# yflyl613/Tiny-NewsRec

Hardware: AMD Instinct MI355X
Metric: training impressions/sec (higher is better)
Workload: dtype fp16; 1 GPU; Tiny-NewsRec 4-layer student (train [2, 3]) + 4-teacher KD (title-emb MSE + soft-CE), fwd+bwd+AMSGrad; batch_per_gpu=32, global_batch=32, user_log_length=50, candidates=5, num_words_title=30, news_dim=256, n_news=51282, parallelism=dp1

## Files before the change

### tiny-newsrec_amd/csrc/attn.hip

```cpp
#include "common.h"

namespace {

constexpr float NEG_BIG = -3.0e38f;
#ifndef TNR_ATTN_TS
#define TNR_ATTN_TS 144
#endif
constexpr int TS = TNR_ATTN_TS;
constexpr int TB = 32 * TS;

__device__ __forceinline__ f32x16 zero16() {
    f32x16 z;
#pragma unroll
    for (int r = 0; r < 16; ++r) z[r] = 0.f;
    return z;
}

__device__ __forceinline__ bf16x8 cat4(bf16x4 a, bf16x4 b) { return __builtin_shufflevector(a, b, 0, 1, 2, 3, 4, 5, 6, 7); }

__device__ __forceinline__ bf16x8 tr_frag(const char* tile, int s, int ct, int lane) {
    const int g16 = lane >> 4, hh = g16 >> 1, i16 = lane & 15, q = i16 >> 2, p = i16 & 3;
    const int row = 16 * s + 4 * hh + q;
    const int col = ct * 32 + 16 * (g16 & 1) + 4 * p;
    bf16x4 v0 = ds_read_tr16(tile + row * TS + col * 2);
    bf16x4 v1 = ds_read_tr16(tile + (row + 8) * TS + col * 2);
    return cat4(v0, v1);
}

__device__ __forceinline__ void acc_to_frags(const f32x16& x, bf16x8 (&f)[2]) {
#pragma unroll
    for (int s = 0; s < 2; ++s)
#pragma unroll
        for (int jj = 0; jj < 8; ++jj) f[s][jj] = (bf16)x[8 * s + jj];
}

__device__ __forceinline__ void acc_to_lds(char* tile, const f32x16& x, int ct, int lane, float scale) {
    const int h = lane >> 5, c = ct * 32 + (lane & 31);
#pragma unroll
    for (int r = 0; r < 16; ++r) {
        int row = (r & 3) + 8 * (r >> 2) + 4 * h;
        *(bf16*)(tile + row * TS + c * 2) = (bf16)(x[r] * scale);
    }
}

__global__ __launch_bounds__(256) void attn_fwd_kernel(const bf16* __restrict__ qkv, const float* __restrict__ mask_add,
                                                       const float* __restrict__ rel, bf16* __restrict__ ctx,
                                                       int64_t n_pairs, int L, int A, TnrDrop drop) {
    __shared__ __attribute__((aligned(16))) char lds[4][TB];
    const int lane = threadIdx.x & 63, w = threadIdx.x >> 6;
    int64_t pair = (int64_t)blockIdx.x * 4 + w;
    const bool valid = pair < n_pairs;
    if (!valid) pair = n_pairs - 1;
    const int64_t n = pair / A;
    const int a = (int)(pair - n * A);
    const int HD = A * 64;
    const int64_t ldq = 3 * HD;
    const int row = lane & 31, h = lane >> 5;
    const int rowc = row < L ? row : L - 1;
    char* my = lds[w];

    f32x4 mkv[4], rlv[4];
    {
        const float* relp0 = rel + a * 1024 + row * 32;
        const float* mp0 = mask_add + n * 32;
#pragma unroll
        for (int g = 0; g < 4; ++g) {
            mkv[g] = *(const f32x4*)(mp0 + 8 * g + 4 * h);
            rlv[g] = *(const f32x4*)(relp0 + 8 * g + 4 * h);
        }
    }
    const bf16* qp = qkv + (n * L + rowc) * ldq + a * 64 + 8 * h;
    bf16x8 qf[4], kf[4];
#pragma unroll
    for (int s = 0; s < 4; ++s) {
        qf[s] = *(const bf16x8*)(qp + 16 * s);
        kf[s] = *(const bf16x8*)(qp + HD + 16 * s);
    }
#pragma unroll
    for (int p = 0; p < 4; ++p) {
        int idx = p * 64 + lane, r = idx >> 3, c = idx & 7;
        int rc = r < L ? r : L - 1;
        *(bf16x8*)(my + r * TS + c * 16) = *(const bf16x8*)(qkv + (n * L + rc) * ldq + 2 * HD + a * 64 + c * 8);
    }
    f32x16 st = zero16();
#pragma unroll
    for (int s = 0; s < 4; ++s) st = TNR_MFMA_32x32x16(kf[s], qf[s], st, 0, 0, 0);

    float mx = NEG_BIG;
#pragma unroll
    for (int g = 0; g < 4; ++g) {
        const f32x4 mk = mkv[g], rl = rlv[g];
#pragma unroll
        for (int e = 0; e < 4; ++e) {
            float v = st[4 * g + e] * 0.125f + mk[e] + rl[e];
            st[4 * g + e] = v;
            mx = fmaxf(mx, v);
        }
    }
    mx = fmaxf(mx, __shfl_xor(mx, 32, 64));
    float sum = 0.f;
#pragma unroll
    for (int r = 0; r < 16; ++r) {
        st[r] = __expf(st[r] - mx);
        sum += st[r];
    }
    sum += __shfl_xor(sum, 32, 64);
    const float inv = 1.0f / sum;
#pragma unroll
    for (int r = 0; r < 16; ++r) st[r] *= inv;
    if (drop.thresh) {
#pragma unroll
        for (int g = 0; g < 4; ++g) {
            float dm[4];
            tnr_drop_prob_row(drop, (uint64_t)pair, 8, row, 8 * g + 4 * h, dm);
#pragma unroll
            for (int e = 0; e < 4; ++e) st[4 * g + e] *= dm[e];
        }
    }
    bf16x8 pf[2];
    acc_to_frags(st, pf);

    f32x16 o[2];
#pragma unroll
    for (int ct = 0; ct < 2; ++ct) {
        o[ct] = zero16();
#pragma unroll
        for (int s = 0; s < 2; ++s)
            o[ct] = TNR_MFMA_32x32x16(pf[s], tr_frag(my, s, ct, lane), o[ct], 0, 0, 0);
    }
    acc_to_lds(my, o[0], 0, lane, 1.0f);
    acc_to_lds(my, o[1], 1, lane, 1.0f);
#pragma unroll
    for (int p = 0; p < 4; ++p) {
        int idx = p * 64 + lane, r = idx >> 3, c = idx & 7;
        if (valid && r < L) *(bf16x8*)(ctx + (n * L + r) * HD + a * 64 + c * 8) = *(const bf16x8*)(my + r * TS + c * 16);
    }
}

__global__ __launch_bounds__(256, 2) void attn_bwd_kernel(const bf16* __restrict__ qkv, const float* __restrict__ mask_add,
                                                       const float* __restrict__ rel, const bf16* __restrict__ dctx,
                                                       bf16* __restrict__ dqkv, float* __restrict__ bias_part,
                                                       int64_t n_pairs, int L, int A, TnrDrop drop) {
    __shared__ __attribute__((aligned(16))) char lds[4][3 * TB + 256];
    const int lane = threadIdx.x & 63, w = threadIdx.x >> 6;
    int64_t pair = (int64_t)blockIdx.x * 4 + w;
    const bool valid = pair < n_pairs;
    if (!valid) pair = n_pairs - 1;
    const int64_t n = pair / A;
    const int a = (int)(pair - n * A);
    const int HD = A * 64;
    const int64_t ldq = 3 * HD;
    const int row = lane & 31, h = lane >> 5;
    const int rowc = row < L ? row : L - 1;
    char* tK = lds[w];
    char* tO = tK + TB;
    char* tQ = tK + 2 * TB;
    float* stat = (float*)(tK + 3 * TB);

    f32x4 mkv[4], rlv[4];
    float relcol[16];
    const float* mp = mask_add + n * 32;
    const float mkcol = mp[row];
    {
        const float* relp0 = rel + a * 1024 + row * 32;
        const float* relc0 = rel + a * 1024 + row;
#pragma unroll
        for (int g = 0; g < 4; ++g) {
            mkv[g] = *(const f32x4*)(mp + 8 * g + 4 * h);
            rlv[g] = *(const f32x4*)(relp0 + 8 * g + 4 * h);
#pragma unroll
            for (int e = 0; e < 4; ++e) relcol[4 * g + e] = relc0[(8 * g + 4 * h + e) * 32];
        }
    }
    const bf16* qp = qkv + (n * L + rowc) * ldq + a * 64 + 8 * h;
    const bf16* dop = dctx + (n * L + rowc) * HD + a * 64 + 8 * h;
    bf16x8 qf[4], kf[4], vf[4], df[4];
#pragma unroll
    for (int s = 0; s < 4; ++s) {
        qf[s] = *(const bf16x8*)(qp + 16 * s);
        kf[s] = *(const bf16x8*)(qp + HD + 16 * s);
        vf[s] = *(const bf16x8*)(qp + 2 * HD + 16 * s);
        df[s] = *(const bf16x8*)(dop + 16 * s);
        if (row >= L) {
#pragma unroll
            for (int e = 0; e < 8; ++e) df[s][e] = (bf16)0.f;
        }
        int off = row * TS + (16 * s + 8 * h) * 2;
        *(bf16x8*)(tK + off) = kf[s];
        *(bf16x8*)(tO + off) = df[s];
        *(bf16x8*)(tQ + off) = qf[s];
    }

    f32x16 st = zero16(), dpt = zero16();
#pragma unroll
    for (int s = 0; s < 4; ++s) {
        st = TNR_MFMA_32x32x16(kf[s], qf[s], st, 0, 0, 0);
        dpt = TNR_MFMA_32x32x16(vf[s], df[s], dpt, 0, 0, 0);
    }
    {
        float mx = NEG_BIG;
#pragma unroll
        for (int g = 0; g < 4; ++g) {
            const f32x4 mk = mkv[g], rl = rlv[g];
#pragma unroll
            for (int e = 0; e < 4; ++e) {
                float v = st[4 * g + e] * 0.125f + mk[e] + rl[e];
                st[4 * g + e] = v;
                mx = fmaxf(mx, v);
            }
        }
        mx = fmaxf(mx, __shfl_xor(mx, 32, 64));
        float sum = 0.f;
#pragma unroll
        for (int r = 0; r < 16; ++r) {
            st[r] = __expf(st[r] - mx);
            sum += st[r];
        }
        sum += __shfl_xor(sum, 32, 64);
        const float inv = 1.0f / sum;
        float dsum = 0.f;
        if (drop.thresh) {
#pragma unroll
            for (int g = 0; g < 4; ++g) {
                float dm[4];
                tnr_drop_prob_row(drop, (uint64_t)pair, 8, row, 8 * g + 4 * h, dm);
#pragma unroll
                for (int e = 0; e < 4; ++e) dpt[4 * g + e] *= dm[e];
            }
        }
#pragma unroll
        for (int r = 0; r < 16; ++r) {
            st[r] *= inv;
            dsum += st[r] * dpt[r];
        }
        dsum += __shfl_xor(dsum, 32, 64);
        if (h == 0) {
            stat[row] = mx + __logf(sum);
            stat[32 + row] = dsum;
        }
#pragma unroll
        for (int r = 0; r < 16; ++r) st[r] = st[r] * (dpt[r] - dsum);
    }
    bf16x8 dstf[2];
    acc_to_frags(st, dstf);
    f32x16 dq[2];
#pragma unroll
    for (int ct = 0; ct < 2; ++ct) {
        dq[ct] = zero16();
#pragma unroll
        for (int s = 0; s < 2; ++s)
            dq[ct] = TNR_MFMA_32x32x16(dstf[s], tr_frag(tK, s, ct, lane), dq[ct], 0, 0, 0);
    }

    f32x16 sn = zero16(), dpn = zero16();
#pragma unroll
    for (int s = 0; s < 4; ++s) {
        sn = TNR_MFMA_32x32x16(qf[s], kf[s], sn, 0, 0, 0);
        dpn = TNR_MFMA_32x32x16(df[s], vf[s], dpn, 0, 0, 0);
    }
    {
        const float mk = mkcol;
#pragma unroll
        for (int g = 0; g < 4; ++g) {
            f32x4 lse = *(const f32x4*)(stat + 8 * g + 4 * h);
            f32x4 dd = *(const f32x4*)(stat + 32 + 8 * g + 4 * h);
            float dm[4] = {1.f, 1.f, 1.f, 1.f};
            if (drop.thresh) tnr_drop_prob_col(drop, (uint64_t)pair, 8, 8 * g + 4 * h, row, dm);
#pragma unroll
            for (int e = 0; e < 4; ++e) {
                float p = __expf(sn[4 * g + e] * 0.125f + mk + relcol[4 * g + e] - lse[e]);
                sn[4 * g + e] = p * dm[e];
                float dpm;
                {
#pragma clang fp contract(off)
                    dpm = dpn[4 * g + e] * dm[e];
                }
                dpn[4 * g + e] = p * (dpm - dd[e]);
            }
        }
    }
    bf16x8 pnf[2], dsf[2];
    acc_to_frags(sn, pnf);
    acc_to_frags(dpn, dsf);
    f32x16 dv[2], dk[2];
#pragma unroll
    for (int ct = 0; ct < 2; ++ct) {
        dv[ct] = zero16();
        dk[ct] = zero16();
#pragma unroll
        for (int s = 0; s < 2; ++s) {
            dv[ct] = TNR_MFMA_32x32x16(pnf[s], tr_frag(tO, s, ct, lane), dv[ct], 0, 0, 0);
            dk[ct] = TNR_MFMA_32x32x16(dsf[s], tr_frag(tQ, s, ct, lane), dk[ct], 0, 0, 0);
        }
    }
    if (bias_part != nullptr && valid) {
        float* bp = bias_part + n * ldq + a * 64 + (lane & 31);
#pragma unroll
        for (int ct = 0; ct < 2; ++ct) {
            float sq = 0.f, sk = 0.f, sv = 0.f;
#pragma unroll
            for (int r = 0; r < 16; ++r) {
                sq += (float)(bf16)(dq[ct][r] * 0.125f);
                sk += (float)(bf16)(dk[ct][r] * 0.125f);
                sv += (float)(bf16)dv[ct][r];
            }
            sq += __shfl_xor(sq, 32, 64);
            sk += __shfl_xor(sk, 32, 64);
            sv += __shfl_xor(sv, 32, 64);
            if (h == 0) {
                bp[ct * 32] = sq;
                bp[HD + ct * 32] = sk;
                bp[2 * HD + ct * 32] = sv;
            }
        }
    }
    acc_to_lds(tK, dq[0], 0, lane, 0.125f);
    acc_to_lds(tK, dq[1], 1, lane, 0.125f);
    acc_to_lds(tO, dk[0], 0, lane, 0.125f);
    acc_to_lds(tO, dk[1], 1, lane, 0.125f);
    acc_to_lds(tQ, dv[0], 0, lane, 1.0f);
    acc_to_lds(tQ, dv[1], 1, lane, 1.0f);
#pragma unroll
    for (int p = 0; p < 4; ++p) {
        int idx = p * 64 + lane, r = idx >> 3, c = idx & 7;
        if (valid && r < L) {
            bf16* dst = dqkv + (n * L + r) * ldq + a * 64 + c * 8;
            *(bf16x8*)(dst) = *(const bf16x8*)(tK + r * TS + c * 16);
            *(bf16x8*)(dst + HD) = *(const bf16x8*)(tO + r * TS + c * 16);
            *(bf16x8*)(dst + 2 * HD) = *(const bf16x8*)(tQ + r * TS + c * 16);
        }
    }
}

__device__ __forceinline__ bf16x8 ld_frag(const bf16* base, int64_t ld, int row, int h, int s) {
    return *(const bf16x8*)(base + (int64_t)row * ld + 16 * s + 8 * h);
}

__global__ __launch_bounds__(256, 3) void attn_long_fwd_kernel(const bf16* __restrict__ qkv, const float* __restrict__ mask_add,
                                                            const float* __restrict__ rel, bf16* __restrict__ ctx,
                                                            float* __restrict__ lse, int64_t n_items, int L, int Lr, int A,
                                                            TnrDrop drop) {
    __shared__ __attribute__((aligned(16))) char sk[2][TB], sv[2][TB], so[4][TB];
    const int tid = threadIdx.x, lane = tid & 63, w = tid >> 6;
    const int nqt = Lr >> 5, nqg = (nqt + 3) >> 2;
    const int qg = (int)(blockIdx.x % nqg);
    const int64_t na = blockIdx.x / nqg;
    (void)n_items;
    const int64_t n = na / A;
    const int a = (int)(na - n * A);
    const int qt_raw = qg * 4 + w;
    const bool valid = qt_raw < nqt;
    const int qt = valid ? qt_raw : nqt - 1;
    const int HD = A * 64;
    const int64_t ldq = 3 * HD;
    const int row = lane & 31, h = lane >> 5;
    char* my = so[w];
    const int qi = qt * 32 + row;
    const int qic = qi < L ? qi : L - 1;
    const bf16* qbase = qkv + (n * L) * ldq + a * 64;
    bf16x8 qf[4];
#pragma unroll
    for (int s = 0; s < 4; ++s) qf[s] = ld_frag(qbase, ldq, qic, h, s);
    f32x16 o[2] = {zero16(), zero16()};
    float m_run = NEG_BIG, l_run = 0.f;
    const float* relq = rel + ((int64_t)a * Lr + (qi < Lr ? qi : Lr - 1)) * Lr;
    const float* mp = mask_add + n * Lr;
    const int lr = tid >> 3, lc = tid & 7;
    bf16x8 kreg, vreg;
    auto gload = [&](int kt) {
        int rc = kt * 32 + lr;
        rc = rc < L ? rc : L - 1;
        kreg = *(const bf16x8*)(qbase + HD + (int64_t)rc * ldq + lc * 8);
        vreg = *(const bf16x8*)(qbase + 2 * HD + (int64_t)rc * ldq + lc * 8);
    };
    f32x4 mkn[4], rln[4];
    auto aload = [&](int kt) {
#pragma unroll
        for (int g = 0; g < 4; ++g) {
            mkn[g] = *(const f32x4*)(mp + kt * 32 + 8 * g + 4 * h);
            rln[g] = *(const f32x4*)(relq + kt * 32 + 8 * g + 4 * h);
        }
    };
    gload(0);
    aload(0);
    for (int kt = 0; kt < nqt; ++kt) {
        const int cur = kt & 1;
        *(bf16x8*)(sk[cur] + lr * TS + lc * 16) = kreg;
        *(bf16x8*)(sv[cur] + lr * TS + lc * 16) = vreg;
        f32x4 mkc[4], rlc[4];
#pragma unroll
        for (int g = 0; g < 4; ++g) { mkc[g] = mkn[g]; rlc[g] = rln[g]; }
        __syncthreads();
        if (kt + 1 < nqt) { gload(kt + 1); aload(kt + 1); }
        bf16x8 kf[4];
#pragma unroll
        for (int s = 0; s < 4; ++s) kf[s] = *(const bf16x8*)(sk[cur] + row * TS + (16 * s + 8 * h) * 2);
        f32x16 st = zero16();
#pragma unroll
        for (int s = 0; s < 4; ++s) st = TNR_MFMA_32x32x16(kf[s], qf[s], st, 0, 0, 0);
        float mx = NEG_BIG;
#pragma unroll
        for (int g = 0; g < 4; ++g) {
            const f32x4 mk = mkc[g], rl = rlc[g];
#pragma unroll
            for (int e = 0; e < 4; ++e) {
                float v = st[4 * g + e] * 0.125f + mk[e] + rl[e];
                st[4 * g + e] = v;
                mx = fmaxf(mx, v);
            }
        }
        mx = fmaxf(mx, __shfl_xor(mx, 32, 64));
        const float m_new = fmaxf(m_run, mx);
        const float alpha = __expf(m_run - m_new);
        float sum = 0.f;
#pragma unroll
        for (int r = 0; r < 16; ++r) {
            st[r] = __expf(st[r] - m_new);
            sum += st[r];
        }
        sum += __shfl_xor(sum, 32, 64);
        l_run = l_run * alpha + sum;
        m_run = m_new;
        if (drop.thresh) {
#pragma unroll
            for (int g = 0; g < 4; ++g) {
                float dm[4];
                tnr_drop_prob_row(drop, (uint64_t)na, Lr >> 2, qi < Lr ? qi : Lr - 1, kt * 32 + 8 * g + 4 * h, dm);
#pragma unroll
                for (int e = 0; e < 4; ++e) st[4 * g + e] *= dm[e];
            }
        }
        bf16x8 pf[2];
        acc_to_frags(st, pf);
#pragma unroll
        for (int ct = 0; ct < 2; ++ct) {
#pragma unroll
            for (int r = 0; r < 16; ++r) o[ct][r] *= alpha;
#pragma unroll
            for (int s = 0; s < 2; ++s) o[ct] = TNR_MFMA_32x32x16(tr_frag(sv[cur], s, ct, lane), pf[s], o[ct], 0, 0, 0);
        }
    }
    const float inv = 1.0f / l_run;
    if (valid && h == 0 && qi < Lr) lse[(n * A + a) * Lr + qi] = m_run + __logf(l_run);
#pragma unroll
    for (int ct = 0; ct < 2; ++ct)
#pragma unroll
        for (int r = 0; r < 16; ++r) {
            int dd = ct * 32 + (r & 3) + 8 * (r >> 2) + 4 * h;
            *(bf16*)(my + row * TS + dd * 2) = (bf16)(o[ct][r] * inv);
        }
#pragma unroll
    for (int p = 0; p < 4; ++p) {
        int idx = p * 64 + lane, r = idx >> 3, c = idx & 7;
        int q = qt * 32 + r;
        if (valid && q < L) *(bf16x8*)(ctx + (n * L + q) * HD + a * 64 + c * 8) = *(const bf16x8*)(my + r * TS + c * 16);
    }
}

__global__ __launch_bounds__(256) void attn_long_bwd_dq_kernel(const bf16* __restrict__ qkv, const float* __restrict__ mask_add,
                                                               const float* __restrict__ rel, const bf16* __restrict__ ctx,
                                                               const bf16* __restrict__ dctx, const float* __restrict__ lse,
                                                               float* __restrict__ delta, bf16* __restrict__ dqkv,
                                                               int64_t n_items, int L, int Lr, int A, TnrDrop drop) {
    __shared__ __attribute__((aligned(16))) char lds[4][TB];
    const int tid = threadIdx.x, lane = tid & 63, w = tid >> 6;
    (void)n_items;
    const int nqt = Lr >> 5, nqg = (nqt + 3) >> 2;
    const int qg = (int)(blockIdx.x % nqg);
    const int64_t na = blockIdx.x / nqg;
    const int64_t n = na / A;
    const int a = (int)(na - n * A);
    const int qt_raw = qg * 4 + w;
    const bool valid = qt_raw < nqt;
    const int qt = valid ? qt_raw : nqt - 1;
    const int HD = A * 64;
    const int64_t ldq = 3 * HD;
    const int row = lane & 31, h = lane >> 5;
    const int qi = qt * 32 + row;
    const int qic = qi < L ? qi : L - 1;
    const bf16* qbase = qkv + (n * L) * ldq + a * 64;
    const bf16* obase = ctx + (n * L) * HD + a * 64;
    const bf16* dobase = dctx + (n * L) * HD + a * 64;
    bf16x8 qf[4], df[4];
    float dl = 0.f;
#pragma unroll
    for (int s = 0; s < 4; ++s) {
        qf[s] = ld_frag(qbase, ldq, qic, h, s);
        df[s] = ld_frag(dobase, HD, qic, h, s);
        bf16x8 of = ld_frag(obase, HD, qic, h, s);
#pragma unroll
        for (int e = 0; e < 8; ++e) dl += (float)df[s][e] * (float)of[e];
        if (qi >= L) {
#pragma unroll
            for (int e = 0; e < 8; ++e) df[s][e] = (bf16)0.f;
        }
    }
    dl += __shfl_xor(dl, 32, 64);
    if (qi >= L) dl = 0.f;
    const float lse_i = lse[(n * A + a) * Lr + (qi < Lr ? qi : Lr - 1)];
    if (valid && h == 0 && qi < Lr) delta[(n * A + a) * Lr + qi] = dl;
    const float* relq = rel + ((int64_t)a * Lr + (qi < Lr ? qi : Lr - 1)) * Lr;
    const float* mp = mask_add + n * Lr;
    f32x16 dq[2] = {zero16(), zero16()};
    const int lr = tid >> 3, lc = tid & 7;
    bf16x8 kreg, vreg;
    auto gload = [&](int kt) {
        int rc = kt * 32 + lr;
        rc = rc < L ? rc : L - 1;
        kreg = *(const bf16x8*)(qbase + HD + (int64_t)rc * ldq + lc * 8);
        vreg = *(const bf16x8*)(qbase + 2 * HD + (int64_t)rc * ldq + lc * 8);
    };
    f32x4 mkn[4], rln[4];
    auto aload = [&](int kt) {
#pragma unroll
        for (int g = 0; g < 4; ++g) {
            mkn[g] = *(const f32x4*)(mp + kt * 32 + 8 * g + 4 * h);
            rln[g] = *(const f32x4*)(relq + kt * 32 + 8 * g + 4 * h);
        }
    };
    gload(0);
    aload(0);
    for (int kt = 0; kt < nqt; ++kt) {
        char* sk = lds[kt & 1];
        char* sv = lds[2 + (kt & 1)];
        *(bf16x8*)(sk + lr * TS + lc * 16) = kreg;
        *(bf16x8*)(sv + lr * TS + lc * 16) = vreg;
        f32x4 mkc[4], rlc[4];
#pragma unroll
        for (int g = 0; g < 4; ++g) { mkc[g] = mkn[g]; rlc[g] = rln[g]; }
        __syncthreads();
        if (kt + 1 < nqt) { gload(kt + 1); aload(kt + 1); }
        bf16x8 kf[4], vf[4];
#pragma unroll
        for (int s = 0; s < 4; ++s) {
            kf[s] = *(const bf16x8*)(sk + row * TS + (16 * s + 8 * h) * 2);
            vf[s] = *(const bf16x8*)(sv + row * TS + (16 * s + 8 * h) * 2);
        }
        f32x16 st = zero16(), dpt = zero16();
#pragma unroll
        for (int s = 0; s < 4; ++s) {
            st = TNR_MFMA_32x32x16(kf[s], qf[s], st, 0, 0, 0);
            dpt = TNR_MFMA_32x32x16(vf[s], df[s], dpt, 0, 0, 0);
        }
#pragma unroll
        for (int g = 0; g < 4; ++g) {
            const f32x4 mk = mkc[g], rl = rlc[g];
            float dm[4] = {1.f, 1.f, 1.f, 1.f};
            if (drop.thresh) tnr_drop_prob_row(drop, (uint64_t)na, Lr >> 2, qi < Lr ? qi : Lr - 1, kt * 32 + 8 * g + 4 * h, dm);
#pragma unroll
            for (int e = 0; e < 4; ++e) {
                float p = __expf(st[4 * g + e] * 0.125f + mk[e] + rl[e] - lse_i);
                st[4 * g + e] = p * (dpt[4 * g + e] * dm[e] - dl);
            }
        }
        bf16x8 dsf[2];
        acc_to_frags(st, dsf);
#pragma unroll
        for (int ct = 0; ct < 2; ++ct)
#pragma unroll
            for (int s = 0; s < 2; ++s) dq[ct] = TNR_MFMA_32x32x16(dsf[s], tr_frag(sk, s, ct, lane), dq[ct], 0, 0, 0);
    }
    __syncthreads();
    char* my = lds[w];
    acc_to_lds(my, dq[0], 0, lane, 0.125f);
    acc_to_lds(my, dq[1], 1, lane, 0.125f);
#pragma unroll
    for (int p = 0; p < 4; ++p) {
        int idx = p * 64 + lane, r = idx >> 3, c = idx & 7;
        int q = qt * 32 + r;
        if (valid && q < L) *(bf16x8*)(dqkv + (n * L + q) * ldq + a * 64 + c * 8) = *(const bf16x8*)(my + r * TS + c * 16);
    }
}

__global__ __launch_bounds__(256, 2) void attn_long_bwd_dkv_kernel(const bf16* __restrict__ qkv, const float* __restrict__ mask_add,
                                                                const float* __restrict__ rel, const bf16* __restrict__ dctx,
                                                                const float* __restrict__ lse, const float* __restrict__ delta,
                                                                bf16* __restrict__ dqkv, int64_t n_items, int L, int Lr, int A,
                                                                TnrDrop drop) {
    __shared__ __attribute__((aligned(16))) char lds[12][TB];
    const int tid = threadIdx.x, lane = tid & 63, w = tid >> 6;
    (void)n_items;
    const int nqt = Lr >> 5, nkg = (nqt + 3) >> 2;
    const int kg = (int)(blockIdx.x % nkg);
    const int64_t na = blockIdx.x / nkg;
    const int64_t n = na / A;
    const int a = (int)(na - n * A);
    const int kt_raw = kg * 4 + w;
    const bool valid = kt_raw < nqt;
    const int kt = valid ? kt_raw : nqt - 1;
    const int HD = A * 64;
    const int64_t ldq = 3 * HD;
    const int row = lane & 31, h = lane >> 5;
    const int kj = kt * 32 + row;
    const int kjc = kj < L ? kj : L - 1;
    const bf16* qbase = qkv + (n * L) * ldq + a * 64;
    const bf16* dobase = dctx + (n * L) * HD + a * 64;
    char* const myK = lds[4 + 2 * w];
    char* const myV = lds[5 + 2 * w];
#pragma unroll
    for (int s = 0; s < 4; ++s) {
        const int off = row * TS + (16 * s + 8 * h) * 2;
        *(bf16x8*)(myK + off) = ld_frag(qbase + HD, ldq, kjc, h, s);
        *(bf16x8*)(myV + off) = ld_frag(qbase + 2 * HD, ldq, kjc, h, s);
    }
    const float mk = mask_add[n * Lr + (kj < Lr ? kj : Lr - 1)];
    const float* relc = rel + (int64_t)a * Lr * Lr + (kj < Lr ? kj : Lr - 1);
    const float* lsep = lse + (n * A + a) * Lr;
    const float* dlp = delta + (n * A + a) * Lr;
    f32x16 dv[2] = {zero16(), zero16()}, dk[2] = {zero16(), zero16()};
    const int lr = tid >> 3, lc = tid & 7;
    bf16x8 qreg, dreg;
    auto gload = [&](int qt) {
        const int q = qt * 32 + lr;
        const int qc = q < L ? q : L - 1;
        qreg = *(const bf16x8*)(qbase + (int64_t)qc * ldq + lc * 8);
        dreg = *(const bf16x8*)(dobase + (int64_t)qc * HD + lc * 8);
        if (q >= L) {
#pragma unroll
            for (int e = 0; e < 8; ++e) dreg[e] = (bf16)0.f;
        }
    };
    gload(0);
    for (int qt = 0; qt < nqt; ++qt) {
        char* tO = lds[qt & 1];
        char* tQ = lds[2 + (qt & 1)];
        *(bf16x8*)(tO + lr * TS + lc * 16) = dreg;
        *(bf16x8*)(tQ + lr * TS + lc * 16) = qreg;
        __syncthreads();
        if (qt + 1 < nqt) gload(qt + 1);
        bf16x8 qf[4], df[4];
#pragma unroll
        for (int s = 0; s < 4; ++s) {
            qf[s] = *(const bf16x8*)(tQ + row * TS + (16 * s + 8 * h) * 2);
            df[s] = *(const bf16x8*)(tO + row * TS + (16 * s + 8 * h) * 2);
        }
        f32x16 sn = zero16(), dpn = zero16();
#pragma unroll
        for (int s = 0; s < 4; ++s) {
            const bf16x8 kfs = *(const bf16x8*)(myK + row * TS + (16 * s + 8 * h) * 2);
            const bf16x8 vfs = *(const bf16x8*)(myV + row * TS + (16 * s + 8 * h) * 2);
            sn = TNR_MFMA_32x32x16(qf[s], kfs, sn, 0, 0, 0);
            dpn = TNR_MFMA_32x32x16(df[s], vfs, dpn, 0, 0, 0);
        }
#pragma unroll
        for (int g = 0; g < 4; ++g) {
            f32x4 ls = *(const f32x4*)(lsep + qt * 32 + 8 * g + 4 * h);
            f32x4 dd = *(const f32x4*)(dlp + qt * 32 + 8 * g + 4 * h);
            float dm[4] = {1.f, 1.f, 1.f, 1.f};
            if (drop.thresh) tnr_drop_prob_col(drop, (uint64_t)na, Lr >> 2, qt * 32 + 8 * g + 4 * h, kj < Lr ? kj : Lr - 1, dm);
#pragma unroll
            for (int e = 0; e < 4; ++e) {
                int q = qt * 32 + 8 * g + 4 * h + e;
                float p = __expf(sn[4 * g + e] * 0.125f + mk + relc[(int64_t)q * Lr] - ls[e]);
                sn[4 * g + e] = p * dm[e];
                dpn[4 * g + e] = p * (dpn[4 * g + e] * dm[e] - dd[e]);
            }
        }
        bf16x8 pnf[2], dsf[2];
        acc_to_frags(sn, pnf);
        acc_to_frags(dpn, dsf);
#pragma unroll
        for (int ct = 0; ct < 2; ++ct)
#pragma unroll
            for (int s = 0; s < 2; ++s) {
                dv[ct] = TNR_MFMA_32x32x16(pnf[s], tr_frag(tO, s, ct, lane), dv[ct], 0, 0, 0);
                dk[ct] = TNR_MFMA_32x32x16(dsf[s], tr_frag(tQ, s, ct, lane), dk[ct], 0, 0, 0);
            }
    }
    __syncthreads();
    char* sK = lds[2 * w];
    char* sV = lds[2 * w + 1];
    acc_to_lds(sK, dk[0], 0, lane, 0.125f);
    acc_to_lds(sK, dk[1], 1, lane, 0.125f);
    acc_to_lds(sV, dv[0], 0, lane, 1.0f);
    acc_to_lds(sV, dv[1], 1, lane, 1.0f);
#pragma unroll
    for (int p = 0; p < 4; ++p) {
        int idx = p * 64 + lane, r = idx >> 3, c = idx & 7;
        int j = kt * 32 + r;
        if (valid && j < L) {
            bf16* dst = dqkv + (n * L + j) * ldq + a * 64 + c * 8;
            *(bf16x8*)(dst + HD) = *(const bf16x8*)(sK + r * TS + c * 16);
            *(bf16x8*)(dst + 2 * HD) = *(const bf16x8*)(sV + r * TS + c * 16);
        }
    }
}

}

extern "C" int TNR_NAME(tnr_attn_l32_fwd)(const void* qkv, const float* mask_add, const float* rel, void* ctx, int64_t n_seq,
                                int L, int A, void* stream) {
    return TNR_NAME(tnr_attn_l32_fwd_do)(qkv, mask_add, rel, ctx, n_seq, L, A, nullptr, stream);
}
extern "C" int TNR_NAME(tnr_attn_l32_fwd_do)(const void* qkv, const float* mask_add, const float* rel, void* ctx, int64_t n_seq,
                                   int L, int A, const tnr_dropout_t* drop, void* stream) {
    TnrDrop dd;
    if (int rc = tnr_make_drop(drop, &dd, "tnr_attn_l32_fwd")) return rc;
    TNR_CHECK_ARG(qkv && mask_add && rel && ctx, "tnr_attn_l32_fwd: null pointer");
    TNR_CHECK_ARG(L >= 1 && L <= 32 && A >= 1 && n_seq >= 1, "tnr_attn_l32_fwd: need 1<=L<=32");
    TNR_CHECK_ARG(((uintptr_t)qkv % 16) == 0 && ((uintptr_t)ctx % 16) == 0, "tnr_attn_l32_fwd: 16-byte alignment");
    int64_t pairs = n_seq * A;
    hipLaunchKernelGGL(attn_fwd_kernel, dim3((unsigned)((pairs + 3) / 4)), dim3(256), 0, (hipStream_t)stream,
                       (const bf16*)qkv, mask_add, rel, (bf16*)ctx, pairs, L, A, dd);
    TNR_CHECK_LAUNCH("tnr_attn_l32_fwd");
    return TNR_OK;
}

extern "C" int TNR_NAME(tnr_attn_l32_bwd)(const void* qkv, const float* mask_add, const float* rel, const void* dctx, void* dqkv,
                                float* bias_part, int64_t n_seq, int L, int A, void* stream) {
    return TNR_NAME(tnr_attn_l32_bwd_do)(qkv, mask_add, rel, dctx, dqkv, bias_part, n_seq, L, A, nullptr, stream);
}
extern "C" int TNR_NAME(tnr_attn_l32_bwd_do)(const void* qkv, const float* mask_add, const float* rel, const void* dctx, void* dqkv,
                                   float* bias_part, int64_t n_seq, int L, int A, const tnr_dropout_t* drop, void* stream) {
    TnrDrop dd;
    if (int rc = tnr_make_drop(drop, &dd, "tnr_attn_l32_bwd")) return rc;
    TNR_CHECK_ARG(qkv && mask_add && rel && dctx && dqkv, "tnr_attn_l32_bwd: null pointer");
    TNR_CHECK_ARG(L >= 1 && L <= 32 && A >= 1 && n_seq >= 1, "tnr_attn_l32_bwd: need 1<=L<=32");
    TNR_CHECK_ARG(((uintptr_t)qkv % 16) == 0 && ((uintptr_t)dctx % 16) == 0 && ((uintptr_t)dqkv % 16) == 0,
                  "tnr_attn_l32_bwd: 16-byte alignment");
    int64_t pairs = n_seq * A;
    hipLaunchKernelGGL(attn_bwd_kernel, dim3((unsigned)((pairs + 3) / 4)), dim3(256), 0, (hipStream_t)stream,
                       (const bf16*)qkv, mask_add, rel, (const bf16*)dctx, (bf16*)dqkv, bias_part, pairs, L, A, dd);
    TNR_CHECK_LAUNCH("tnr_attn_l32_bwd");
    return TNR_OK;
}

extern "C" int TNR_NAME(tnr_attn_long_fwd)(const void* qkv, const float* mask_add, const float* rel, void* ctx, float* lse,
                                           int64_t n_seq, int L, int A, void* stream) {
    return TNR_NAME(tnr_attn_long_fwd_do)(qkv, mask_add, rel, ctx, lse, n_seq, L, A, nullptr, stream);
}
extern "C" int TNR_NAME(tnr_attn_long_fwd_do)(const void* qkv, const float* mask_add, const float* rel, void* ctx, float* lse,
                                              int64_t n_seq, int L, int A, const tnr_dropout_t* drop, void* stream) {
    TnrDrop dd;
    if (int rc = tnr_make_drop(drop, &dd, "tnr_attn_long_fwd")) return rc;
    TNR_CHECK_ARG(qkv && mask_add && rel && ctx && lse, "tnr_attn_long_fwd: null pointer");
    TNR_CHECK_ARG(L >= 1 && L <= 512 && A >= 1 && n_seq >= 1, "tnr_attn_long_fwd: need 1<=L<=512");
    TNR_CHECK_ARG(((uintptr_t)qkv % 16) == 0 && ((uintptr_t)ctx % 16) == 0, "tnr_attn_long_fwd: 16-byte alignment");
    const int Lr = (L + 31) / 32 * 32;
    int64_t items = n_seq * A * (Lr / 32);
    const int64_t blocks = n_seq * A * ((Lr / 32 + 3) / 4);
    hipLaunchKernelGGL(attn_long_fwd_kernel, dim3((unsigned)blocks), dim3(256), 0, (hipStream_t)stream,
                       (const bf16*)qkv, mask_add, rel, (bf16*)ctx, lse, items, L, Lr, A, dd);
    TNR_CHECK_LAUNCH("tnr_attn_long_fwd");
    return TNR_OK;
}

extern "C" int TNR_NAME(tnr_attn_long_bwd)(const void* qkv, const float* mask_add, const float* rel, const void* ctx,
                                           const void* dctx, const float* lse, float* delta, void* dqkv, int64_t n_seq,
                                           int L, int A, void* stream) {
    return TNR_NAME(tnr_attn_long_bwd_do)(qkv, mask_add, rel, ctx, dctx, lse, delta, dqkv, n_seq, L, A, nullptr, stream);
}
extern "C" int TNR_NAME(tnr_attn_long_bwd_do)(const void* qkv, const float* mask_add, const float* rel, const void* ctx,
                                              const void* dctx, const float* lse, float* delta, void* dqkv, int64_t n_seq,
                                              int L, int A, const tnr_dropout_t* drop, void* stream) {
    TnrDrop dd;
    if (int rc = tnr_make_drop(drop, &dd, "tnr_attn_long_bwd")) return rc;
    TNR_CHECK_ARG(qkv && mask_add && rel && ctx && dctx && lse && delta && dqkv, "tnr_attn_long_bwd: null pointer");
    TNR_CHECK_ARG(L >= 1 && L <= 512 && A >= 1 && n_seq >= 1, "tnr_attn_long_bwd: need 1<=L<=512");
    TNR_CHECK_ARG(((uintptr_t)qkv % 16) == 0 && ((uintptr_t)ctx % 16) == 0 && ((uintptr_t)dctx % 16) == 0 &&
                  ((uintptr_t)dqkv % 16) == 0, "tnr_attn_long_bwd: 16-byte alignment");
    const int Lr = (L + 31) / 32 * 32;
    int64_t items = n_seq * A * (Lr / 32);
    dim3 grid((unsigned)(n_seq * A * ((Lr / 32 + 3) / 4))), blk(256);
    hipLaunchKernelGGL(attn_long_bwd_dq_kernel, grid, blk, 0, (hipStream_t)stream, (const bf16*)qkv, mask_add, rel,
                       (const bf16*)ctx, (const bf16*)dctx, lse, delta, (bf16*)dqkv, items, L, Lr, A, dd);
    TNR_CHECK_LAUNCH("tnr_attn_long_bwd/dq");
    hipLaunchKernelGGL(attn_long_bwd_dkv_kernel, grid, blk, 0, (hipStream_t)stream, (const bf16*)qkv, mask_add, rel,
                       (const bf16*)dctx, lse, delta, (bf16*)dqkv, items, L, Lr, A, dd);
    TNR_CHECK_LAUNCH("tnr_attn_long_bwd/dkv");
    return TNR_OK;
}
```

Measured before the change: 4226 impressions/s.

## Skip K/V loads for masked keys and stage rel bias through LDS in backward

The forward and backward attention kernels now compute a per-pair mask of live keys with a ballot over the additive mask, and load K and V rows only for keys not masked out. Masked keys get zeros, which should be numerically equivalent because their softmax weight is already negligible. The backward kernel also loads the 32x32 relative-position bias with coalesced vector reads into a new LDS tile, then reads the row and column views from LDS instead of doing strided global gathers. The forward kernel gets a min-blocks-per-CU launch bound of 5. The backward LDS footprint grows by one tile per wave, which may lower occupancy.

```diff
diff --git a/tiny-newsrec_amd/csrc/attn.hip b/tiny-newsrec_amd/csrc/attn.hip
--- a/tiny-newsrec_amd/csrc/attn.hip
+++ b/tiny-newsrec_amd/csrc/attn.hip
@@ -14,6 +14,31 @@
 #pragma unroll
     for (int r = 0; r < 16; ++r) z[r] = 0.f;
     return z;
+}
+
+__device__ __forceinline__ bf16x8 zero8() {
+    bf16x8 z;
+#pragma unroll
+    for (int e = 0; e < 8; ++e) z[e] = (bf16)0.f;
+    return z;
+}
+
+#ifndef TNR_ATTN_LOAD_DEAD_KEYS
+#define TNR_ATTN_LOAD_DEAD_KEYS 0
+#endif
+__device__ __forceinline__ uint32_t live_keys(const f32x4 (&mkv)[4], float mk_own) {
+#if TNR_ATTN_LOAD_DEAD_KEYS
+    return 0xFFFFFFFFu;
+#else
+    constexpr float DEAD_BELOW = -9000.f;
+    float mx = NEG_BIG;
+#pragma unroll
+    for (int g = 0; g < 4; ++g)
+#pragma unroll
+        for (int e = 0; e < 4; ++e) mx = fmaxf(mx, mkv[g][e]);
+    mx = fmaxf(mx, __shfl_xor(mx, 32, 64));
+    return (uint32_t)__ballot(!(mk_own - mx <= DEAD_BELOW));
+#endif
 }
 
 __device__ __forceinline__ bf16x8 cat4(bf16x4 a, bf16x4 b) { return __builtin_shufflevector(a, b, 0, 1, 2, 3, 4, 5, 6, 7); }
@@ -43,7 +68,7 @@
     }
 }
 
-__global__ __launch_bounds__(256) void attn_fwd_kernel(const bf16* __restrict__ qkv, const float* __restrict__ mask_add,
+__global__ __launch_bounds__(256, 5) void attn_fwd_kernel(const bf16* __restrict__ qkv, const float* __restrict__ mask_add,
                                                        const float* __restrict__ rel, bf16* __restrict__ ctx,
                                                        int64_t n_pairs, int L, int A, TnrDrop drop) {
     __shared__ __attribute__((aligned(16))) char lds[4][TB];
@@ -60,9 +85,10 @@
     char* my = lds[w];
 
     f32x4 mkv[4], rlv[4];
+    const float* mp0 = mask_add + n * 32;
+    const float mkown = mp0[row];
     {
         const float* relp0 = rel + a * 1024 + row * 32;
-        const float* mp0 = mask_add + n * 32;
 #pragma unroll
         for (int g = 0; g < 4; ++g) {
             mkv[g] = *(const f32x4*)(mp0 + 8 * g + 4 * h);
@@ -74,13 +100,20 @@
 #pragma unroll
     for (int s = 0; s < 4; ++s) {
         qf[s] = *(const bf16x8*)(qp + 16 * s);
-        kf[s] = *(const bf16x8*)(qp + HD + 16 * s);
+        kf[s] = zero8();
+    }
+    const uint32_t live = live_keys(mkv, mkown);
+    if ((live >> row) & 1) {
+#pragma unroll
+        for (int s = 0; s < 4; ++s) kf[s] = *(const bf16x8*)(qp + HD + 16 * s);
     }
 #pragma unroll
     for (int p = 0; p < 4; ++p) {
         int idx = p * 64 + lane, r = idx >> 3, c = idx & 7;
         int rc = r < L ? r : L - 1;
-        *(bf16x8*)(my + r * TS + c * 16) = *(const bf16x8*)(qkv + (n * L + rc) * ldq + 2 * HD + a * 64 + c * 8);
+        bf16x8 vr = zero8();
+        if ((live >> r) & 1) vr = *(const bf16x8*)(qkv + (n * L + rc) * ldq + 2 * HD + a * 64 + c * 8);
+        *(bf16x8*)(my + r * TS + c * 16) = vr;
     }
     f32x16 st = zero16();
 #pragma unroll
@@ -141,7 +174,7 @@
                                                        const float* __restrict__ rel, const bf16* __restrict__ dctx,
                                                        bf16* __restrict__ dqkv, float* __restrict__ bias_part,
                                                        int64_t n_pairs, int L, int A, TnrDrop drop) {
-    __shared__ __attribute__((aligned(16))) char lds[4][3 * TB + 256];
+    __shared__ __attribute__((aligned(16))) char lds[4][4 * TB + 256];
     const int lane = threadIdx.x & 63, w = threadIdx.x >> 6;
     int64_t pair = (int64_t)blockIdx.x * 4 + w;
     const bool valid = pair < n_pairs;
@@ -156,31 +189,36 @@
     char* tO = tK + TB;
     char* tQ = tK + 2 * TB;
     float* stat = (float*)(tK + 3 * TB);
-
+    char* tR = tK + 3 * TB + 256;
+
+    f32x4 rst[4];
+#pragma unroll
+    for (int p = 0; p < 4; ++p) rst[p] = *(const f32x4*)(rel + a * 1024 + (p * 64 + lane) * 4);
     f32x4 mkv[4], rlv[4];
     float relcol[16];
     const float* mp = mask_add + n * 32;
     const float mkcol = mp[row];
-    {
-        const float* relp0 = rel + a * 1024 + row * 32;
-        const float* relc0 = rel + a * 1024 + row;
-#pragma unroll
-        for (int g = 0; g < 4; ++g) {
-            mkv[g] = *(const f32x4*)(mp + 8 * g + 4 * h);
-            rlv[g] = *(const f32x4*)(relp0 + 8 * g + 4 * h);
-#pragma unroll
-            for (int e = 0; e < 4; ++e) relcol[4 * g + e] = relc0[(8 * g + 4 * h + e) * 32];
-        }
-    }
+#pragma unroll
+    for (int g = 0; g < 4; ++g) mkv[g] = *(const f32x4*)(mp + 8 * g + 4 * h);
     const bf16* qp = qkv + (n * L + rowc) * ldq + a * 64 + 8 * h;
     const bf16* dop = dctx + (n * L + rowc) * HD + a * 64 + 8 * h;
     bf16x8 qf[4], kf[4], vf[4], df[4];
 #pragma unroll
     for (int s = 0; s < 4; ++s) {
         qf[s] = *(const bf16x8*)(qp + 16 * s);
-        kf[s] = *(const bf16x8*)(qp + HD + 16 * s);
-        vf[s] = *(const bf16x8*)(qp + 2 * HD + 16 * s);
         df[s] = *(const bf16x8*)(dop + 16 * s);
+        kf[s] = zero8();
+        vf[s] = zero8();
+    }
+    if ((live_keys(mkv, mkcol) >> row) & 1) {
+#pragma unroll
+        for (int s = 0; s < 4; ++s) {
+            kf[s] = *(const bf16x8*)(qp + HD + 16 * s);
+            vf[s] = *(const bf16x8*)(qp + 2 * HD + 16 * s);
+        }
+    }
+#pragma unroll
+    for (int s = 0; s < 4; ++s) {
         if (row >= L) {
 #pragma unroll
             for (int e = 0; e < 8; ++e) df[s][e] = (bf16)0.f;
@@ -189,6 +227,17 @@
         *(bf16x8*)(tK + off) = kf[s];
         *(bf16x8*)(tO + off) = df[s];
         *(bf16x8*)(tQ + off) = qf[s];
+    }
+#pragma unroll
+    for (int p = 0; p < 4; ++p) {
+        int idx = p * 64 + lane, r = idx >> 3, c = idx & 7;
+        *(f32x4*)(tR + r * TS + c * 16) = rst[p];
+    }
+#pragma unroll
+    for (int g = 0; g < 4; ++g) {
+        rlv[g] = *(const f32x4*)(tR + row * TS + (8 * g + 4 * h) * 4);
+#pragma unroll
+        for (int e = 0; e < 4; ++e) relcol[4 * g + e] = *(const float*)(tR + (8 * g + 4 * h + e) * TS + row * 4);
     }
 
     f32x16 st = zero16(), dpt = zero16();
```

New measurement: 4281 impressions/s (median of 6 runs). 1.01x the previous value.
